# jimsnow/glome

Hardware: AMD Instinct MI355X
Metric: Mrays/sec + fps at 1920x1080 primary+shadow; 1/2/4/8 MI355X (higher is better)
Workload: dtype f32; 1 GPU; S3: 100,352-triangle heightfield under bih (BASELINE configs[2]), 1 light, primary + shadow rays, maxdepth 1; width=1920, height=1080, sampling=renderTile, 1 primary ray/pixel, launches_in_flight=4, frames_per_launch=32, transport=none (one GPU), frame_product=packed 0x00RRGGBB framebuffer (trace + blitTile fused, 4 B/pixel), bih_build=device (glome_sb_bih_dev / glome_sb_mesh_dev) for lists of 4096+ objects, device_bytes=14337708

## Files before the change

glome_amd/csrc/cull_kernels.hpp:

```cpp
#pragma once
#include <hip/hip_runtime.h>

#include "kernel_launch.hpp"
#include "rt_device.hpp"
#include "tiles.hpp"

constexpr int kCullThreads = 512;
constexpr int kCullWaves = kCullThreads / 64;
constexpr int kCullProbeLane = 36;
constexpr int kScanChunks = 1024, kScanPerThread = kScanChunks / kCullThreads, kScanPerWave = kScanChunks / kCullWaves;
static_assert(kCullThreads % 64 == 0 && kScanPerThread * kCullThreads == kScanChunks && kQueueChunk == 64, "a chunk's live mask is one 64-bit word, a lane per position");

__device__ __forceinline__ void chunk_position(const DRenderArgs& A, uint32_t g, uint32_t& frame, uint32_t& first) {
  frame = 0;
  if (A.chunks_per_frame) {
    const uint32_t nf = (uint32_t)A.nframes, q = g / nf;
    frame = g - q * nf;
    g = q;
  }
  first = g * kQueueChunk;
}

__device__ __forceinline__ DItem ld_item(const DItem* p, uint32_t i) {
#if defined(__HIP_DEVICE_COMPILE__)
  return as_global(p)[i];
#else
  return p[i];
#endif
}

__device__ __forceinline__ bool lane_enters(const DScene& S, const Ray& r, bool valid) {
  bool in = false;
  for (uint32_t e = 0; e < S.n_entries; e++) {
    const U4 w = ld_walk_u(S.walk, e);
    if (w.x & RF_NOVIS) continue;
    const F4 h0 = ld4u(S.bihhdr, 3 * w.y), h1 = ld4u(S.bihhdr, 3 * w.y + 1);
    if (uni(as_u(h0.w)) & BREF_LEAF) return true;
    float nearv, farv;
    bih_root_interval(r, h0, h1, kInf, nearv, farv);
    bih_clip_root_at_origin(nearv);
    in = in || bih_root_enters(valid, nearv, farv);
  }
  return in;
}
__device__ __forceinline__ bool item_live(const DScene& S, const Ray& r, bool valid) { return wave_ballot(lane_enters(S, r, valid)) != 0; }

__global__ void __launch_bounds__(kCullThreads) k_cull_items(DRenderArgs, uint32_t* list, uint32_t* masks, uint32_t nchunks) {
  const DRenderArgs& A = kernel_args<DRenderArgs>();
  __shared__ uint32_t s_bits[2], s_todo[2], s_last, s_wave[kCullWaves];
  const uint32_t tid = threadIdx.x, lane = tid & 63u, wave = uni(tid >> 6), g = blockIdx.x;
  uint32_t frame, first;
  chunk_position(A, g, frame, first);
  const uint32_t npos = min((uint32_t)kQueueChunk, A.total_waves - first);
  const DCamera cam = frame == 0 ? A.cam : A.more_cams[frame - 1];

  if (wave == 0) {
    const bool pos = lane < npos;
    const DItem it = ld_item(A.items, first + (pos ? lane : 0u));
    int px = 0, py = 0;
    size_t dense_off = 0;
    if (!item_pixel(it, A.tiles, kCullProbeLane, px, py, dense_off)) (void)item_pixel(it, A.tiles, 0, px, py, dense_off);
    const Ray ray = primary_ray(cam, ldf(A.xc_tab, (uint32_t)px), ldf(A.yc_tab, (uint32_t)py));
    const LaneMask proven = wave_ballot(pos && lane_enters(A.S, ray, pos));
    const LaneMask todo = wave_ballot(pos) & ~proven;
    if (lane == 0) {
      s_bits[0] = (uint32_t)proven; s_bits[1] = (uint32_t)(proven >> 32);
      s_todo[0] = (uint32_t)todo; s_todo[1] = (uint32_t)(todo >> 32);
    }
  }
  __syncthreads();

  const LaneMask todo = (LaneMask)uni(s_todo[0]) | ((LaneMask)uni(s_todo[1]) << 32);
  LaneMask mine = wave_ballot(((todo >> lane) & 1ull) != 0 && (uint32_t)__builtin_popcountll(todo & ((1ull << lane) - 1ull)) % (uint32_t)kCullWaves == wave);
  LaneMask found = 0;
  uint32_t dead_px = 0;
  for (; mine; mine &= mine - 1ull) {
    const uint32_t j = (uint32_t)__builtin_ctzll(mine);
    const DItem it = ld_item_u(A.items, first + j);
    int px = 0, py = 0;
    size_t dense_off = 0;
    const bool valid = item_pixel(it, A.tiles, (int)lane, px, py, dense_off);
    const float xc = ldf(A.xc_tab, valid ? (uint32_t)px : 0u), yc = ldf(A.yc_tab, valid ? (uint32_t)py : 0u);
    const Ray ray = primary_ray(cam, xc, yc);
    if (item_live(A.S, ray, valid)) {
      found |= 1ull << j;
    } else {
      dead_px += (uint32_t)__builtin_popcountll(wave_ballot(valid));
      float depth = kInf;
      asm volatile("" : "+v"(depth));
      if (valid) store_pixel(A, frame, px, py, dense_off, ca(0, 0, 0, 0), depth);
    }
  }
  if (found && lane == 0) {
    if ((uint32_t)found) atomicOr(&s_bits[0], (uint32_t)found);
    if ((uint32_t)(found >> 32)) atomicOr(&s_bits[1], (uint32_t)(found >> 32));
  }
  if (A.want_counters && dead_px && lane == 0) atomicAdd(&A.counters->rays_primary, (unsigned long long)dead_px);
  __syncthreads();
  if (tid == 0) {
    __hip_atomic_store(&masks[2 * g], s_bits[0], __ATOMIC_RELAXED, __HIP_MEMORY_SCOPE_AGENT);
    __hip_atomic_store(&masks[2 * g + 1], s_bits[1], __ATOMIC_RELAXED, __HIP_MEMORY_SCOPE_AGENT);
    asm volatile("s_waitcnt vmcnt(0)" ::: "memory");
    s_last = atomicAdd(&A.counters->cull_done, 1u) == nchunks - 1u ? 1u : 0u;
  }
  __syncthreads();
  if (!s_last) return;

  uint32_t running = 0;
  for (uint32_t base = 0; base < nchunks; base += (uint32_t)kScanChunks) {
    uint32_t lo[kScanPerThread], hi[kScanPerThread], cnt = 0;
#pragma unroll
    for (int p = 0; p < kScanPerThread; p++) {
      const uint32_t c = base + tid * (uint32_t)kScanPerThread + (uint32_t)p;
      lo[p] = 0; hi[p] = 0;
      if (c < nchunks) {
        lo[p] = __hip_atomic_load(&masks[2 * c], __ATOMIC_RELAXED, __HIP_MEMORY_SCOPE_AGENT);
        hi[p] = __hip_atomic_load(&masks[2 * c + 1], __ATOMIC_RELAXED, __HIP_MEMORY_SCOPE_AGENT);
      }
      cnt += (uint32_t)__builtin_popcount(lo[p]) + (uint32_t)__builtin_popcount(hi[p]);
    }
    uint32_t incl = cnt;
    for (int o = 1; o < 64; o <<= 1) { const uint32_t v = __shfl_up(incl, o, 64); if ((int)lane >= o) incl += v; }
    if (lane == 63) s_wave[wave] = incl;
    __syncthreads();
    uint32_t before = 0, total = 0;
    for (uint32_t w = 0; w < (uint32_t)kCullWaves; w++) { const uint32_t v = s_wave[w]; total += v; if (w < wave) before += v; }
    uint32_t off[kScanPerThread];
    off[0] = running + before + incl - cnt;
#pragma unroll
    for (int p = 1; p < kScanPerThread; p++) off[p] = off[p - 1] + (uint32_t)__builtin_popcount(lo[p - 1]) + (uint32_t)__builtin_popcount(hi[p - 1]);
    uint32_t ck = base + wave * (uint32_t)kScanPerWave, cframe = 0, cfirst = 0;
    if (ck < nchunks) chunk_position(A, ck, cframe, cfirst);
    cframe = uni(cframe); cfirst = uni(cfirst);
    for (uint32_t l = 0; l < 64u && ck < nchunks; l++) {
#pragma unroll
      for (int p = 0; p < kScanPerThread; p++, ck++) {
        const unsigned long long m = (unsigned long long)(uint32_t)__builtin_amdgcn_readlane((int)lo[p], (int)l) | ((unsigned long long)(uint32_t)__builtin_amdgcn_readlane((int)hi[p], (int)l) << 32);
        if (m != 0) {
          const uint32_t o = (uint32_t)__builtin_amdgcn_readlane((int)off[p], (int)l);
          if ((m >> lane) & 1ull) list[o + (uint32_t)__builtin_popcountll(m & ((1ull << lane) - 1ull))] = (cframe << kListFrameShift) | (cfirst + lane);
        }
        if (A.chunks_per_frame && ++cframe != (uint32_t)A.nframes) continue;
        cframe = 0; cfirst += kQueueChunk;
      }
    }
    running += total;
    __syncthreads();
  }
  if (tid == 0) {
    __hip_atomic_store(&A.counters->list_len, running, __ATOMIC_RELAXED, __HIP_MEMORY_SCOPE_AGENT);
    __hip_atomic_store(&A.counters->cull_done, 0u, __ATOMIC_RELAXED, __HIP_MEMORY_SCOPE_AGENT);
  }
}
```

Measured before the change: 36280 Mrays/s.

## Add conservative interval test to prove whole cull items miss the scene

Adds a per-item interval-arithmetic test that bounds the ray directions over a tile's pixel rectangle and checks them against each BIH root box, with ulp widening to stay conservative. Items proven dead skip the per-lane ray test and are blanked directly, with all 64 pixels assumed valid. This is meant to cut the per-lane ray tests in the cull kernel for empty regions, at the cost of extra interval math in wave 0. If few items are provably dead, that extra math adds overhead.

Result: no change. 36330 Mrays/s, median of 6 (+0.1%).

```diff
diff --git a/glome_amd/csrc/cull_interval.hpp b/glome_amd/csrc/cull_interval.hpp
--- /dev/null
+++ b/glome_amd/csrc/cull_interval.hpp
@@ -0,0 +1,80 @@
+#pragma once
+#include <cfloat>
+#include <cstdint>
+
+#include "rt_device.hpp"
+
+namespace glome {
+
+constexpr int kWiden = 16;
+
+GD float cull_step(float x, int n) {
+  const uint32_t b = as_u(x);
+  int32_t key = (b & 0x80000000u) ? -(int32_t)(b & 0x7fffffffu) : (int32_t)b;
+  key += n;
+  return as_f(key < 0 ? (0x80000000u | (uint32_t)(-key)) : (uint32_t)key);
+}
+GD bool cull_finite(float x) { return (as_u(x) & 0x7f800000u) != 0x7f800000u; }
+GD float cull_min(float a, float b) { return a < b ? a : b; }
+GD float cull_max(float a, float b) { return a > b ? a : b; }
+GD float cull_abs(float a) { return as_f(as_u(a) & 0x7fffffffu); }
+GD float cull_len2(float x, float y, float z) { return (x * x) + (y * y) + (z * z); }
+
+GD void cull_dir_bounds(float fwd, float right, float up, float xc_lo, float xc_hi, float yc_lo, float yc_hi, float& u_lo, float& u_hi) {
+  const float a0 = right * (-xc_lo), a1 = right * (-xc_hi), b0 = up * yc_lo, b1 = up * yc_hi;
+  u_lo = fwd + cull_min(a0, a1) + cull_min(b0, b1);
+  u_hi = fwd + cull_max(a0, a1) + cull_max(b0, b1);
+}
+
+GD bool cull_axis(float u_lo, float u_hi, float inv_lo, float inv_hi, float o, float lo, float hi, float& in_lb, float& out_ub) {
+  float d_lo, d_hi;
+  if (u_lo > 0) { d_lo = u_lo * inv_lo; d_hi = u_hi * inv_hi; }
+  else if (u_hi < 0) { d_lo = u_lo * inv_hi; d_hi = u_hi * inv_lo; }
+  else return false;
+  const bool pos = d_lo > 0;
+  if (!pos && !(d_hi < 0)) return false;
+  const float r_lo = cull_step(dir_rcp(d_hi), -kWiden), r_hi = cull_step(dir_rcp(d_lo), kWiden);
+  if (!cull_finite(r_lo) || !cull_finite(r_hi) || !(pos ? r_lo > 0 : r_hi < 0)) return false;
+  const float p_in = (pos ? lo : hi) - o, p_out = (pos ? hi : lo) - o;
+  in_lb = cull_min(p_in * r_lo, p_in * r_hi);
+  out_ub = cull_max(p_out * r_lo, p_out * r_hi);
+  return cull_finite(in_lb) && cull_finite(out_ub);
+}
+
+GD bool item_certainly_dead(const DScene& S, const DCamera& cam, float xc_lo, float xc_hi, float yc_lo, float yc_hi) {
+  float u_lo[3], u_hi[3], m[3], M[3];
+#pragma unroll
+  for (int k = 0; k < 3; k++) {
+    cull_dir_bounds(cam.fwd[k], cam.right[k], cam.up[k], xc_lo, xc_hi, yc_lo, yc_hi, u_lo[k], u_hi[k]);
+    if (!cull_finite(u_lo[k]) || !cull_finite(u_hi[k])) return false;
+    const float al = cull_abs(u_lo[k]), ah = cull_abs(u_hi[k]);
+    M[k] = cull_max(al, ah);
+    m[k] = (u_lo[k] > 0 || u_hi[k] < 0) ? cull_min(al, ah) : 0.0f;
+  }
+  const float len2_lo = cull_len2(m[0], m[1], m[2]), len2_hi = cull_len2(M[0], M[1], M[2]);
+  if (!(len2_lo > 0) || !cull_finite(len2_hi)) return false;
+  const float inv_lo = cull_step(1.0f / sqrtf(len2_hi), -kWiden), inv_hi = cull_step(1.0f / sqrtf(len2_lo), kWiden);
+  if (!cull_finite(inv_lo) || !cull_finite(inv_hi) || !(inv_lo > 0)) return false;
+  for (uint32_t e = 0; e < S.n_entries; e++) {
+    const U4 w = ld_walk_u(S.walk, e);
+    if (w.x & RF_NOVIS) continue;
+    const F4 h0 = ld4u(S.bihhdr, 3 * w.y), h1 = ld4u(S.bihhdr, 3 * w.y + 1);
+    if (uni(as_u(h0.w)) & BREF_LEAF) return false;
+    float in_x, out_x, in_y, out_y, in_z, out_z;
+    if (!cull_axis(u_lo[0], u_hi[0], inv_lo, inv_hi, cam.pos[0], h0.x, h1.x, in_x, out_x)) return false;
+    if (!cull_axis(u_lo[1], u_hi[1], inv_lo, inv_hi, cam.pos[1], h0.y, h1.y, in_y, out_y)) return false;
+    if (!cull_axis(u_lo[2], u_hi[2], inv_lo, inv_hi, cam.pos[2], h0.z, h1.z, in_z, out_z)) return false;
+    const float near_lb = cull_max(-FLT_MIN, cull_max(in_x, cull_max(in_y, in_z)));
+    const float far_ub = cull_min(out_x, cull_min(out_y, out_z));
+    if (!(near_lb > far_ub)) return false;
+  }
+  return true;
+}
+
+GD bool item_certainly_dead(const DScene& S, const DCamera& cam, const DItem& it, const float* xc_tab, const float* yc_tab) {
+  if (it.pitch == kItemStrip) return false;
+  const float xa = ldf(xc_tab, it.x), xb = ldf(xc_tab, it.x + (uint32_t)kBlockW - 1u), ya = ldf(yc_tab, it.y), yb = ldf(yc_tab, it.y + (uint32_t)kBlockH - 1u);
+  return item_certainly_dead(S, cam, cull_min(xa, xb), cull_max(xa, xb), cull_min(ya, yb), cull_max(ya, yb));
+}
+
+}
diff --git a/glome_amd/csrc/cull_kernels.hpp b/glome_amd/csrc/cull_kernels.hpp
--- a/glome_amd/csrc/cull_kernels.hpp
+++ b/glome_amd/csrc/cull_kernels.hpp
@@ -1,6 +1,7 @@
 #pragma once
 #include <hip/hip_runtime.h>
 
+#include "cull_interval.hpp"
 #include "kernel_launch.hpp"
 #include "rt_device.hpp"
 #include "tiles.hpp"
@@ -47,7 +48,7 @@
 
 __global__ void __launch_bounds__(kCullThreads) k_cull_items(DRenderArgs, uint32_t* list, uint32_t* masks, uint32_t nchunks) {
   const DRenderArgs& A = kernel_args<DRenderArgs>();
-  __shared__ uint32_t s_bits[2], s_todo[2], s_last, s_wave[kCullWaves];
+  __shared__ uint32_t s_bits[2], s_todo[2], s_dead[2], s_last, s_wave[kCullWaves];
   const uint32_t tid = threadIdx.x, lane = tid & 63u, wave = uni(tid >> 6), g = blockIdx.x;
   uint32_t frame, first;
   chunk_position(A, g, frame, first);
@@ -62,18 +63,38 @@
     if (!item_pixel(it, A.tiles, kCullProbeLane, px, py, dense_off)) (void)item_pixel(it, A.tiles, 0, px, py, dense_off);
     const Ray ray = primary_ray(cam, ldf(A.xc_tab, (uint32_t)px), ldf(A.yc_tab, (uint32_t)py));
     const LaneMask proven = wave_ballot(pos && lane_enters(A.S, ray, pos));
-    const LaneMask todo = wave_ballot(pos) & ~proven;
+    const LaneMask open = wave_ballot(pos) & ~proven;
+    bool certain = false;
+    if (lane_of(open)) certain = item_certainly_dead(A.S, cam, it, A.xc_tab, A.yc_tab);
+    const LaneMask dead = wave_ballot(certain), todo = open & ~dead;
     if (lane == 0) {
       s_bits[0] = (uint32_t)proven; s_bits[1] = (uint32_t)(proven >> 32);
       s_todo[0] = (uint32_t)todo; s_todo[1] = (uint32_t)(todo >> 32);
+      s_dead[0] = (uint32_t)dead; s_dead[1] = (uint32_t)(dead >> 32);
     }
   }
   __syncthreads();
 
+  float blank_depth = kInf;
+  asm volatile("" : "+v"(blank_depth));
+  uint32_t dead_px = 0;
+
+  const LaneMask dead = (LaneMask)uni(s_dead[0]) | ((LaneMask)uni(s_dead[1]) << 32);
+  if (dead) {
+    LaneMask blank = wave_ballot(((dead >> lane) & 1ull) != 0 && (uint32_t)__builtin_popcountll(dead & ((1ull << lane) - 1ull)) % (uint32_t)kCullWaves == wave);
+    for (; blank; blank &= blank - 1ull) {
+      const DItem it = ld_item_u(A.items, first + (uint32_t)__builtin_ctzll(blank));
+      int px = 0, py = 0;
+      size_t dense_off = 0;
+      (void)item_pixel(it, A.tiles, (int)lane, px, py, dense_off);
+      store_pixel(A, frame, px, py, dense_off, ca(0, 0, 0, 0), blank_depth);
+      dead_px += 64u;
+    }
+  }
+
   const LaneMask todo = (LaneMask)uni(s_todo[0]) | ((LaneMask)uni(s_todo[1]) << 32);
   LaneMask mine = wave_ballot(((todo >> lane) & 1ull) != 0 && (uint32_t)__builtin_popcountll(todo & ((1ull << lane) - 1ull)) % (uint32_t)kCullWaves == wave);
   LaneMask found = 0;
-  uint32_t dead_px = 0;
   for (; mine; mine &= mine - 1ull) {
     const uint32_t j = (uint32_t)__builtin_ctzll(mine);
     const DItem it = ld_item_u(A.items, first + j);
@@ -86,9 +107,7 @@
       found |= 1ull << j;
     } else {
       dead_px += (uint32_t)__builtin_popcountll(wave_ballot(valid));
-      float depth = kInf;
-      asm volatile("" : "+v"(depth));
-      if (valid) store_pixel(A, frame, px, py, dense_off, ca(0, 0, 0, 0), depth);
+      if (valid) store_pixel(A, frame, px, py, dense_off, ca(0, 0, 0, 0), blank_depth);
     }
   }
   if (found && lane == 0) {
```
